# tsurumeso/vocal-remover

Hardware: NVIDIA H100
Metric: seconds-of-audio/sec separated (n_fft=2048, hop=1024) (higher is better)
Workload: dtype bf16x3 (split-bf16 operands hi+lo, 3 wgmma passes, fp32 accumulate); fft/lstm fp32

## Files before the change

### vocal-remover_b200/csrc/api.cu

```cuda
#include <stdio.h>
#include <string.h>

#include <string>

#include "../../include/vr_b200.h"
#include "engine.h"
#include "kernels.h"
#include "tc_plan.h"

struct vr_ctx {
  vr::Engine* eng;
  std::string err;
};

static std::string g_create_err;

static int fail(vr_ctx* c, const std::string& m) {
  if (c) c->err = m;
  return -1;
}
static int done(vr_ctx* c, bool ok) {
  if (ok) return 0;
  c->err = c->eng->err;
  return -1;
// ... 345 lines not shown
  return 0;
}

int64_t vr_launch_count(const vr_ctx* ctx) { return ctx && ctx->eng ? ctx->eng->launches : 0; }

int vr_profile_enable(vr_ctx* ctx, int32_t on) {
  CHECK_CTX(ctx);
  ctx->eng->profile_enable(on != 0);
  return 0;
}

int vr_profile_read(vr_ctx* ctx, double* out6) {
  CHECK_CTX(ctx);
  return done(ctx, ctx->eng->profile_read(out6));
}

int vr_profile_dump(vr_ctx* ctx, char* text, int64_t cap, int64_t* needed) {
  CHECK_CTX(ctx);
  std::string t;
  if (!ctx->eng->profile_dump(t)) return done(ctx, false);
  if (needed) *needed = (int64_t)t.size() + 1;
  if (text && cap > 0) {
    const size_t n = t.size() < (size_t)cap - 1 ? t.size() : (size_t)cap - 1;
    memcpy(text, t.data(), n);
    text[n] = 0;
  }
  return 0;
}

int vr_debug_conv(vr_ctx* ctx, const float* x, int32_t N, int32_t Cin, int32_t H, int32_t W, const float* w,
                  const float* bias, int32_t Cout, int32_t k, int32_t stride, int32_t dil_h, int32_t dil_w, int32_t act,
                  int32_t use_tc, float* y, void* stream) {
  CHECK_CTX(ctx);
  return done(ctx, ctx->eng->debug_conv(x, N, Cin, H, W, w, bias, Cout, k, stride, dil_h, dil_w, act, use_tc, y,
                                        (cudaStream_t)stream));
}

int vr_debug_decoder(vr_ctx* ctx, const float* low, int32_t N, int32_t Cl, int32_t h, int32_t w, const float* skip,
                     int32_t Cs, const float* wgt, const float* bias, int32_t Cout, int32_t act, int32_t fused, float* y,
                     void* stream) {
  CHECK_CTX(ctx);
  return done(ctx, ctx->eng->debug_decoder(low, N, Cl, h, w, skip, Cs, wgt, bias, Cout, act, fused, y,
                                           (cudaStream_t)stream));
}

int vr_debug_tensor(vr_ctx* ctx, const char* name, int32_t n0, int32_t n, float* out, int64_t* shape4, void* stream) {
  CHECK_NET(ctx);
  if (!name || !shape4) return fail(ctx, "vr_debug_tensor: name and shape4 are required");
  return done(ctx, ctx->eng->debug_tensor(name, n0, n, out, shape4, (cudaStream_t)stream));
}

int vr_debug_set(int32_t key, int32_t value) {
  int* knob = key == 0 ? &vr::g_debug.trace : key == 2 ? &vr::g_debug.rows_wide : key == 3 ? &vr::g_debug.halo
            : key == 6 ? &vr::g_debug.kskip : key == 7 ? &vr::g_debug.crop_mask : nullptr;
  if (!knob) return -1;
  *knob = value;
  return 0;
}

int64_t vr_debug_trace(uint64_t* host_out, int64_t capacity) {
  return vr::tc_rows_read_trace((unsigned long long*)host_out, (long long)capacity);
}

}
```

### vocal-remover_b200/csrc/conv_tc.cu

```cuda
#include <cuda.h>
#include <stdio.h>

#include <map>
#include <tuple>

#include "engine.h"
#include "tc_common.cuh"
#include "tc_plan.h"

namespace vr {

static constexpr int kMaxStages = 8;
static constexpr int kConsumerWarps = 8;
static constexpr int kThreads = 32 * kConsumerWarps + 32;
static constexpr int kStaticSmem = 2048;

struct TcParams {
  int N, Ho, Wo, Wt, Ht, Nt, tiles_w, tiles_h, m_tiles, n_tiles;
  int stride, pad_h, pad_w, dil_h, dil_w, KW;
  int cchunks, total_sub, CinPadTC, Cout, act, stages;
  bf16* out_hi;
  bf16* out_lo;
  int64_t osn, osh;
  int osw;
// ... 258 lines not shown

static unsigned long long weight_group_mask(const ConvLayer& L, const float* wp, int CinPad) {
  if (CinPad / 8 > 64) return ~0ull;
  unsigned long long m = 0x3ull;
  for (int ci = 0; ci < L.CinPad; ++ci) {
    bool any = false;
    for (int t = 0; t < L.k * L.k && !any; ++t)
      for (int co = 0; co < L.Cout && !any; ++co) any = wp[((size_t)t * L.CinPad + ci) * L.CoutPad + co] != 0.f;
    if (any) m |= 1ull << (ci / 8);
  }
  return m;
}

static bool encode_weight_map(TcConv& tc, int rows, int K, int box_rows, std::string& err, const std::string& name) {
  cuuint64_t dims[3] = {(cuuint64_t)K, (cuuint64_t)rows, 2};
  cuuint64_t strides[2] = {(cuuint64_t)K * 2, (cuuint64_t)rows * K * 2};
  cuuint32_t box[3] = {(cuuint32_t)tc.KB, (cuuint32_t)box_rows, 2};
  cuuint32_t es[3] = {1, 1, 1};
  CUresult r = tc_encode_fn()(&tc.map_b, CU_TENSOR_MAP_DATA_TYPE_BFLOAT16, 3, tc.w_planes.get(), dims, strides, box, es,
                              CU_TENSOR_MAP_INTERLEAVE_NONE, swizzle_for(tc.KB), CU_TENSOR_MAP_L2_PROMOTION_L2_256B,
                              CU_TENSOR_MAP_FLOAT_OOB_FILL_NONE);
  if (r != CUDA_SUCCESS) {
    err = "cuTensorMapEncodeTiled(weights) failed for " + name + " code " + std::to_string((int)r);
    return false;
  }
  return true;
}

const CUtensorMap* tc_activation_map(TcConv& tc, const ActView& v, int bw, int bh, int bn, int es, std::string& err,
                                     const std::string& name) {
  const ViewKey key = std::make_tuple((const void*)v.hi, (const void*)v.lo, v.N, v.H, v.W, v.C, bw, bh, bn);
  auto it = tc.map_a.find(key);
  if (it != tc.map_a.end()) return &it->second;
  const int64_t plane = (const char*)v.lo - (const char*)v.hi;
  if (v.sw % 8 || v.sh % 8 || v.sn % 8 || (reinterpret_cast<uintptr_t>(v.hi) & 15) || plane <= 0 || plane % 16) {
    err = "internal: the input of " + name + " is not 16-byte aligned or its lo plane does not follow its hi plane";
    return nullptr;
  }
  cuuint64_t dims[5] = {(cuuint64_t)v.C, (cuuint64_t)v.W, (cuuint64_t)v.H, (cuuint64_t)v.N, 2};
  cuuint64_t strides[4] = {(cuuint64_t)v.sw * 2, (cuuint64_t)v.sh * 2, (cuuint64_t)v.sn * 2, (cuuint64_t)plane};
  cuuint32_t box[5] = {(cuuint32_t)tc.KB, (cuuint32_t)bw, (cuuint32_t)bh, (cuuint32_t)bn, 2};
  cuuint32_t estr[5] = {1, (cuuint32_t)es, (cuuint32_t)es, 1, 1};
  CUtensorMap m;
  CUresult r = tc_encode_fn()(&m, CU_TENSOR_MAP_DATA_TYPE_BFLOAT16, 5, (void*)v.hi, dims, strides, box, estr,
                              CU_TENSOR_MAP_INTERLEAVE_NONE, swizzle_for(tc.KB), CU_TENSOR_MAP_L2_PROMOTION_L2_256B,
                              CU_TENSOR_MAP_FLOAT_OOB_FILL_NONE);
  if (r != CUDA_SUCCESS) {
    err = "cuTensorMapEncodeTiled(activations) failed for " + name + " code " + std::to_string((int)r);
    return nullptr;
  }
  return &tc.map_a.emplace(key, m).first->second;
}

bool tc_prepare(ConvLayer& L, const float* w, const float* b, int H, int W, bool rows_wide, std::string& err) {
  const TcKind kind = tc_choose(L, H, W, rows_wide);
  if (kind == TC_NONE) return true;
  if (!tc_encode_fn()) {
    err = "cuTensorMapEncodeTiled is not available from the driver";
    return false;
  }
  auto tc = std::make_shared<TcConv>();
  tc->kind = kind;
  tc->H = H; tc->W = W;
  const NTiling nt = n_tiling(L, kind == TC_ROWS, rows_wide);
  const int BN = nt.BN, cin16 = round_up(L.CinPad, 16);
  tc->BN = BN; tc->n_tiles = nt.n_tiles;
  tc->KB = kind != TC_GENERIC ? 32 : cin16 % 64 == 0 ? 64 : cin16 % 32 == 0 ? 32 : 16;
  const int CinPad = round_up(L.CinPad, tc->KB);
  tc->CinPad = CinPad;
  tc->chunks = CinPad / tc->KB;
  tc->kmask = weight_group_mask(L, w, CinPad);
  const int rows = nt.n_tiles * BN;
  std::vector<uint16_t> planes;
  int brows, K;
  if (kind == TC_ROWS) {
    brows = 3 * rows;
    K = 3 * CinPad;
    planes = split_bf16(L, w, brows, K, [&](int co, int t, int ci) {
      return (size_t)(co / BN * 3 * BN + (2 - t / 3) * BN + co % BN) * K + (size_t)(t % 3) * CinPad + ci;
    });
  } else {
    brows = rows;
    K = L.k * L.k * CinPad;
    planes = split_bf16(L, w, brows, K, [&](int co, int t, int ci) { return (size_t)co * K + (size_t)t * CinPad + ci; });
  }
  std::vector<float> bias((size_t)rows, 0.f);
  for (int co = 0; co < L.Cout; ++co) bias[(size_t)co] = b[co];
  if (tc->w_planes.alloc(planes.size() * 2) != cudaSuccess || tc->bias.alloc(bias.size() * 4) != cudaSuccess) {
    err = "cudaMalloc failed while packing tensor-core weights for " + L.name;
    return false;
  }
  if (!upload(tc->w_planes.get(), planes.data(), planes.size() * 2, err) ||
      !upload(tc->bias.get(), bias.data(), bias.size() * 4, err) ||
      !encode_weight_map(*tc, brows, K, kind == TC_ROWS ? 3 * BN : BN, err, L.name))
    return false;
  L.tc = tc;
  return true;
}

cudaError_t tc_launch(const ConvLayer& L, const ActView& in, const ActView& out, cudaStream_t s, std::string& err,
                      const ConvFusion& f) {
  TcConv& tc = *L.tc;
  if (out.H != tc.H || out.W != tc.W || (in.H - 1) / L.stride + 1 != out.H || (in.W - 1) / L.stride + 1 != out.W) {
    err = "internal: " + L.name + " is launched on maps of another size than it was prepared for";
    return cudaErrorInvalidValue;
  }
// ... 52 lines not shown
```

### vocal-remover_b200/csrc/conv_tc_rows.cu

```cuda
#include <stdio.h>

#include "engine.h"
#include "tc_common.cuh"
#include "tc_plan.h"

namespace vr {

static constexpr int kInterpWarps = 10;
static constexpr int kConsumerWarps = 8;
static constexpr int kTmaWarp = kConsumerWarps;
static constexpr int kInterpWarp0 = kConsumerWarps + 1;
__host__ __device__ constexpr int rows_per_tile(int BN) { return BN == 64 ? 2 : BN == 32 ? 4 : 8; }
static constexpr int kUpProducerWarps = 12;
static constexpr int kUpConsumerRegs = 128;
static constexpr int kUpProducerRegs = 72;
static constexpr int kUpLaunchRegs = 96;
static_assert(kConsumerWarps * kUpConsumerRegs + kUpProducerWarps * kUpProducerRegs <=
                  (kConsumerWarps + kUpProducerWarps) * kUpLaunchRegs,
              "setmaxnreg.inc would wait forever for registers the block does not own");
__host__ __device__ constexpr int rows_threads(bool up) { return 32 * (kConsumerWarps + (up ? kUpProducerWarps : 1)); }
static constexpr int kRowPx = 130;
static constexpr int kBoxPx = 136;
static constexpr int kMaxASlots = 8;
static constexpr int kStaticSmem = 3072;
static constexpr int kSrcPx = 68;
static constexpr uint32_t kKB = 32;
static constexpr uint32_t kRowB = kKB * 2;
static constexpr uint32_t kAPlane = kBoxPx * kRowB;
static constexpr uint32_t kASlot = 2 * kAPlane;

static constexpr int kTraceEvents = 2048;
__device__ unsigned long long g_rows_trace[3 * kTraceEvents * 3];

template <int BN>
struct RowsGeom {
  static constexpr uint32_t kBPlane = 3 * BN * kRowB;
  static constexpr uint32_t kBKw = 2 * kBPlane;
  static constexpr uint32_t kBBuf = 3 * kBKw;
};

struct RowsParams {
  int N, H, W, tiles_w, tiles_h, n_tiles, total_tiles;
  int col0;
  int chunks, CinPadR, Cout, act;
  int n_aslots;
  bf16* out_hi;
  bf16* out_lo;
  int64_t osn, osh;
  int osw;
  const float* bias;
  int up_chunks, xH, xW;
  const bf16* x_hi;
  const bf16* x_lo;
  int64_t xsn, xsh;
  int xsw;
  int trace;
  unsigned long long kmask;
  int a_c_off;
  int l_chunk;
  int n_uslots;
  float up_sh, up_sw;
  const float* dot_w;
  float* dot_out;
  MaskOutParams mask;
};

struct RowsTile {
  int nt, w0, h0, n;
};
template <int R>
__device__ __forceinline__ RowsTile rows_tile(const RowsParams& p, int tile) {
  RowsTile t;
  t.nt = tile % p.n_tiles;
  int mt = tile / p.n_tiles;
  t.w0 = p.col0 + (mt % p.tiles_w) * 128;
  mt /= p.tiles_w;
  t.h0 = (mt % p.tiles_h) * R;
  t.n = mt / p.tiles_h;
  return t;
}

struct RowsConsumer {
  MbarRing a_up, a_tma, b;
  HeldSlot held_b;
};

template <int BN, int R, int r>
__device__ __forceinline__ MbarRing consume_rows(MbarRing a, RowsConsumer& st, float* acc, uint32_t (&fr)[2][16],
                                                 uint32_t lrow, uint32_t bsrc, uint32_t dhi, uint32_t ksm, int lane) {
  constexpr int o_lo = r - 2 < 0 ? 0 : r - 2;
  constexpr int o_hi = r > R - 1 ? R - 1 : r;
  a.wait_full();
  const uint32_t row = lrow + (uint32_t)a.slot * kASlot;
#pragma unroll
  for (int kw = 0; kw < 3; ++kw) {
    uint32_t* f = fr[(3 * r + kw) & 1];
    const uint32_t q = (row >> 6) + (uint32_t)kw;
#pragma unroll
// ... 15 lines not shown
                            b_row + (RowsGeom<BN>::kBPlane >> 4), dhi);
      }
    }
    wg_commit();
    if (kw == 2) warp_arrive(a.empty(), lane);
    wg_wait<1>();
    st.held_b.release(st.b, lane);
  }
  a.advance();
  if constexpr (r + 1 < R + 2)
    return consume_rows<BN, R, r + 1>(a, st, acc, fr, lrow, bsrc, dhi, ksm, lane);
  else
    return a;
}

__device__ __forceinline__ float dot_pair(float v0, float v1, const float* bias_s, const float* dot_s, int c, float slope) {
  const float t0 = v0 + bias_s[c], t1 = v1 + bias_s[c + 1];
  return fmaf(fmaxf(t0, 0.f) + slope * fminf(t0, 0.f), dot_s[c], (fmaxf(t1, 0.f) + slope * fminf(t1, 0.f)) * dot_s[c + 1]);
}

template <int BN>
__device__ __forceinline__ void mask_pixel(const RowsParams& p, const float* v, const float* bias_s,
                                           const float* mask_s, float slope, int lane, int n, int bin, int w) {
  float x[BN / 4];
#pragma unroll
  for (int j = 0; j < BN / 8; ++j) {
    const int c = 8 * j + 2 * (lane & 3);
    const float t0 = v[4 * j] + bias_s[c], t1 = v[4 * j + 1] + bias_s[c + 1];
    const float y0 = fmaxf(t0, 0.f) + slope * fminf(t0, 0.f);
    const float y1 = fmaxf(t1, 0.f) + slope * fminf(t1, 0.f);
    const float2 hf = bf2_to_f2(f2_to_bf2(y0, y1));
    const float2 lf = bf2_to_f2(f2_to_bf2(y0 - hf.x, y1 - hf.y));
    x[2 * j] = hf.x + lf.x;
    x[2 * j + 1] = hf.y + lf.y;
  }
  const float* wm = mask_s + (lane & 1) * BN;
  float a = 0.f;
#pragma unroll
  for (int c = 0; c < BN; ++c)
    a = fmaf(__shfl_sync(0xffffffffu, x[2 * (c >> 3) + (c & 1)], (lane & ~3) | ((c >> 1) & 3)), wm[c], a);
  const float m = 1.f / (1.f + expf(-a));
  const int tr = w - p.col0;
  const int64_t t = p.mask.t_base0 + (int64_t)n * p.mask.roi_t + tr;
  const bool nyquist = (lane & 2) != 0;
  if (t < 0 || t >= p.mask.t_limit || (nyquist && bin != p.H - 1)) return;
  float* d = p.mask.out + (int64_t)n * p.mask.stride_n + (int64_t)(nyquist ? bin + 1 : bin) * p.mask.stride_bin +
             p.mask.t_base0 + tr + ((lane & 1) ? p.mask.stride_c : 0);
  *d = p.mask.accumulate ? (*d + m) * 0.5f : m;
}

template <int BN, bool UP>
__global__ void __launch_bounds__(rows_threads(UP), 1)
    conv_tc_rows_kernel(const __grid_constant__ CUtensorMap tmA, const __grid_constant__ CUtensorMap tmB,
                        const __grid_constant__ CUtensorMap tmL, const RowsParams p) {
  typedef RowsGeom<BN> G;
  constexpr int R = rows_per_tile(BN);
  extern __shared__ uint8_t smem_raw[];
  __shared__ __align__(8) uint64_t bar_afull[kMaxASlots];
  __shared__ __align__(8) uint64_t bar_aempty[kMaxASlots];
  __shared__ __align__(8) uint64_t bar_bfull[2];
  __shared__ __align__(8) uint64_t bar_bempty[2];
  __shared__ float bias_s[256];
  __shared__ float dot_s[256];

  const int warp = __shfl_sync(0xffffffffu, (int)threadIdx.x >> 5, 0);
  const int lane = threadIdx.x & 31;
  const uint32_t smem_base = (smem_u32(smem_raw) + 1023u) & ~1023u;
  const uint32_t a_base = smem_base;
  const uint32_t b_base = smem_base + (uint32_t)p.n_aslots * kASlot;
  MbarRing a_up(smem_u32(&bar_afull[0]), smem_u32(&bar_aempty[0]), 0, p.n_uslots);
  MbarRing a_tma(smem_u32(&bar_afull[0]), smem_u32(&bar_aempty[0]), p.n_uslots, p.n_aslots);
  MbarRing b_ring(smem_u32(&bar_bfull[0]), smem_u32(&bar_bempty[0]), 0, 2);

  if (warp == kTmaWarp && lane == 0) {
    tma_prefetch(&tmA);
    tma_prefetch(&tmB);
    a_up.init(kInterpWarps, kConsumerWarps);
    a_tma.init(1, kConsumerWarps);
    b_ring.init(1, kConsumerWarps);
    asm volatile("fence.mbarrier_init.release.cluster;" ::: "memory");
  }
  for (int i = threadIdx.x; i < p.n_tiles * BN; i += blockDim.x) {
    bias_s[i] = __ldg(p.bias + i);
    dot_s[i] = p.dot_out && i < p.Cout ? __ldg(p.dot_w + i) : 0.f;
  }
  constexpr bool kMaskable = UP && BN <= 32;
  if constexpr (kMaskable) {
    if (p.mask.out)
      for (int i = threadIdx.x; i < 2 * BN; i += blockDim.x) dot_s[i] = __ldg(p.mask.w + i);
  }
  __syncthreads();
  if (warp < kConsumerWarps) {
    if constexpr (UP) setmaxnreg_inc<kUpConsumerRegs>();
    const int wg = warp >> 2;
    const float slope = act_slope(p.act);
    const uint32_t dhi = desc_hi(8 * kRowB, 2u);
    const uint32_t lrow = a_base + (uint32_t)(64 * wg + 16 * (warp & 3) + (lane & 15)) * kRowB;
    RowsConsumer st{a_up, a_tma, b_ring};
    float acc[R * BN / 2];
    uint32_t fr[2][16];
    for (int tile = blockIdx.x; tile < p.total_tiles; tile += gridDim.x) {
#pragma unroll
      for (int i = 0; i < R * BN / 2; ++i) acc[i] = 0.f;
      for (int cc = 0; cc < p.chunks; ++cc) {
        st.b.wait_full();
        const uint32_t bsrc = desc_lo(b_base + (uint32_t)st.b.slot * G::kBBuf);
        const bool up = cc < p.up_chunks;
        const uint32_t gm = chunk_groups(p.kmask, cc);
        const uint32_t ksm = ((gm & 0x3u) ? 1u : 0u) | ((gm & 0xCu) ? 2u : 0u);
        const MbarRing a = consume_rows<BN, R, 0>(up ? st.a_up : st.a_tma, st, acc, fr, lrow, bsrc, dhi, ksm, lane);
        st.a_up.slot = up ? a.slot : st.a_up.slot;
        st.a_up.phase = up ? a.phase : st.a_up.phase;
        st.a_tma.slot = up ? st.a_tma.slot : a.slot;
        st.a_tma.phase = up ? st.a_tma.phase : a.phase;
        st.held_b.hold(st.b);
        st.b.advance();
      }
      wg_wait<0>();
      st.held_b.release_last(st.b, lane);

      const RowsTile tl = rows_tile<R>(p, tile);
      const int w0 = tl.w0, h0 = tl.h0, n = tl.n;
      const int c_lane = tl.nt * BN + 2 * (lane & 3);
#pragma unroll
      for (int orow = 0; orow < R; ++orow) {
#pragma unroll
        for (int hr = 0; hr < 2; ++hr) {
          const int px = 64 * wg + 16 * (warp & 3) + (lane >> 2) + 8 * hr;
          const float* v = acc + orow * (BN / 2) + 2 * hr;
          if constexpr (kMaskable) {
            if (p.mask.out) {
              mask_pixel<BN>(p, v, bias_s, dot_s, slope, lane, n, h0 + orow, w0 + px);
              continue;
            }
          }
          if (p.dot_out) {
            float d = 0.f;
#pragma unroll
            for (int j = 0; j < BN / 8; ++j) d += dot_pair(v[4 * j], v[4 * j + 1], bias_s, dot_s, c_lane + 8 * j, slope);
            d += __shfl_xor_sync(0xffffffffu, d, 1);
            d += __shfl_xor_sync(0xffffffffu, d, 2);
            if ((lane & 3) == 0) atomicAdd(p.dot_out + ((int64_t)n * p.H + (h0 + orow)) * p.W + (w0 + px), d);
          }
          const int64_t obase = (int64_t)n * p.osn + (int64_t)(h0 + orow) * p.osh + (int64_t)(w0 + px) * p.osw;
#pragma unroll
          for (int j = 0; j < BN / 8; ++j)
            epilogue_pair(v[4 * j], v[4 * j + 1], bias_s, c_lane + 8 * j, p.Cout, slope, p.out_hi + obase,
                          p.out_lo + obase);
        }
      }
    }
  } else {
    if constexpr (UP) setmaxnreg_dec<kUpProducerRegs>();
    if (warp == kTmaWarp) {
      if (elect_one_sync()) {
#ifdef VR_TRACE
        const bool tr = p.trace && blockIdx.x == 0;
#else
        constexpr bool tr = false;
#endif
        int tn = 0;
        for (int tile = blockIdx.x; tile < p.total_tiles; tile += gridDim.x) {
          const RowsTile tl = rows_tile<R>(p, tile);
          const int nt = tl.nt, w0 = tl.w0, h0 = tl.h0, n = tl.n;
          for (int cc = 0; cc < p.chunks; ++cc) {
            b_ring.wait_empty();
            const uint32_t bdst = b_base + (uint32_t)b_ring.slot * G::kBBuf;
            mbar_expect_tx(b_ring.full(), G::kBBuf);
#pragma unroll
            for (int kw = 0; kw < 3; ++kw)
              tma_load_3d(bdst + (uint32_t)kw * G::kBKw, &tmB, kw * p.CinPadR + cc * (int)kKB, nt * 3 * BN, 0,
                          b_ring.full());
            b_ring.advance();
            if (cc < p.up_chunks) continue;
            const bool from_l = cc == p.l_chunk;
            const int c0 = from_l ? 0 : cc * (int)kKB + p.a_c_off;
            for (int r = 0; r < R + 2; ++r) {
              const unsigned long long t0 = tr ? clock64() : 0ull;
              a_tma.wait_empty();
              mbar_expect_tx(a_tma.full(), kASlot);
              tma_load_5d(a_base + (uint32_t)a_tma.slot * kASlot, from_l ? &tmL : &tmA, c0, w0 - 1, h0 - 1 + r, n, 0,
                          a_tma.full());
              if (tr && tn < kTraceEvents) {
                g_rows_trace[(1 * kTraceEvents + tn) * 3 + 0] = t0;
                g_rows_trace[(1 * kTraceEvents + tn) * 3 + 1] = clock64();
                g_rows_trace[(1 * kTraceEvents + tn) * 3 + 2] = 0ull;
                ++tn;
              }
              a_tma.advance();
            }
          }
        }
      }
      __syncwarp();
    } else if (UP && warp < kInterpWarp0 + kInterpWarps) {
      if (p.up_chunks > 0) {
        const int wk = warp - kInterpWarp0;
        const int xi = lane >> 2, j = lane & 3;
        const int sx = 7 * wk + xi;
        const bool emit = xi < 7 && sx < kSrcPx;
        const float inv_sw = p.up_sw > 0.f ? 1.f / p.up_sw : 0.f;
#ifdef VR_TRACE
        const bool tr = p.trace && blockIdx.x == 0 && wk == 0;
#else
// ... 94 lines not shown
#pragma unroll
              for (int i = 0; i < 8; ++i) {
                const float t = __shfl_down_sync(0xffffffffu, v[i], 4);
                nv[i] = last_px ? v[i] : t;
              }
              const unsigned long long t1 = tr ? clock64() : 0ull;
              a_up.wait_empty();
              const unsigned long long t2 = tr ? clock64() : 0ull;
              uint8_t* slot = smem_raw + (a_base - smem_u32(smem_raw)) + (size_t)a_up.slot * kASlot;
#pragma unroll
              for (int k = 0; k < 3; ++k) {
                if (e_off[k] < 0) continue;
                const float lx = e_lx[k], hx = 1.f - lx;
                float y[8];
#pragma unroll
                for (int i = 0; i < 8; ++i) y[i] = hx * v[i] + lx * nv[i];
                bf16x8 oh, ol;
                split8(y, oh, ol);
                *reinterpret_cast<uint4*>(slot + e_off[k]) = oh;
                *reinterpret_cast<uint4*>(slot + kAPlane + e_off[k]) = ol;
              }
              if (z_off >= 0) {
                *reinterpret_cast<uint4*>(slot + z_off) = make_uint4(0, 0, 0, 0);
                *reinterpret_cast<uint4*>(slot + kAPlane + z_off) = make_uint4(0, 0, 0, 0);
              }
              warp_arrive(a_up.full(), lane);
              fetch();
              if (tr && lane == 0 && tn < kTraceEvents) {
                g_rows_trace[(2 * kTraceEvents + tn) * 3 + 0] = t0;
                g_rows_trace[(2 * kTraceEvents + tn) * 3 + 1] = t2 - t1;
                g_rows_trace[(2 * kTraceEvents + tn) * 3 + 2] = clock64();
              }
              ++tn;
              a_up.advance();
            }
          }
        }
      }
      }
  }
}

#define VR_ROWS_FOR_ALL(X) X(16, true) X(16, false) X(32, true) X(32, false) X(64, true) X(64, false)

static int rows_b_bytes(int BN) {
#define VR_ROWS_B(BN_, UP_) if (BN == BN_) return (int)(2 * RowsGeom<BN_>::kBBuf);
  VR_ROWS_FOR_ALL(VR_ROWS_B)
#undef VR_ROWS_B
  return 0;
}

bool tc_rows_has(int BN) { return rows_b_bytes(BN) > 0; }

cudaError_t tc_rows_launch(const ConvLayer& L, TcConv& tc, const ActView& in, const ActView& out, cudaStream_t s,
                           std::string& err, const ConvFusion& f) {
  const ActView* up_src = f.up;
  if (up_src && (!tc.fuses_upsample(up_src->C) || up_src->H * 2 != in.H || up_src->W * 2 != in.W || up_src->sw % 8)) {
    err = "tc_rows_launch: fused upsample needs a half-resolution source of 32k channels";
    return cudaErrorInvalidValue;
  }
  if (up_src && up_src->C + in.C > tc.CinPad) {
    err = "tc_rows_launch: with a fused upsample the input must hold only the channels after the up-sampled ones";
    return cudaErrorInvalidValue;
  }
  const ActView* last = f.last_chunk;
  if (last && (last->H != in.H || last->W != in.W || last->N != in.N || last->C > tc.KB)) {
    err = "tc_rows_launch: the last-chunk tensor must match the input geometry and fit one chunk";
    return cudaErrorInvalidValue;
  }
  const CUtensorMap* map_a = tc_activation_map(tc, in, kBoxPx, 1, 1, 1, err, L.name);
  const CUtensorMap* map_l = last ? tc_activation_map(tc, *last, kBoxPx, 1, 1, 1, err, L.name) : map_a;
  if (!map_a || !map_l) return cudaErrorInvalidValue;
  if (f.mask && !tc.fuses_mask(L.Cout, f.mask->offset, up_src != nullptr)) {
    err = "tc_rows_launch: the fused output layer needs a fused upsample, one N tile of Cout <= 32 channels and a "
          "kept width that is a multiple of 128";
    return cudaErrorInvalidValue;
  }
  const int col0 = f.mask ? f.mask->offset : 0;
  RowsParams p;
  p.N = out.N; p.H = out.H; p.W = out.W;
  const bool up = up_src != nullptr;
  p.col0 = col0;
  p.tiles_w = (out.W - 2 * col0) / 128; p.tiles_h = out.H / rows_per_tile(tc.BN); p.n_tiles = tc.n_tiles;
  p.total_tiles = p.tiles_w * p.tiles_h * out.N * tc.n_tiles;
  p.chunks = tc.chunks; p.CinPadR = tc.CinPad; p.Cout = L.Cout; p.act = L.act;
  p.out_hi = out.hi; p.out_lo = out.lo;
  p.osn = out.sn; p.osh = out.sh; p.osw = out.sw;
  p.bias = tc.bias.get();
  p.up_chunks = 0; p.xH = p.xW = 0;
  p.x_hi = p.x_lo = nullptr; p.xsn = p.xsh = 0; p.xsw = 0;
  p.trace = g_debug.trace == 1 ? 1 : 0;
  p.up_sh = p.up_sw = 0.f;
  p.dot_w = f.dot_w; p.dot_out = f.dot_w ? f.dot_out : nullptr;
  p.mask = f.mask ? *f.mask : MaskOutParams{};
  p.a_c_off = 0;
  p.l_chunk = last ? tc.chunks - 1 : -1;
  p.kmask = g_debug.kskip == 1 ? tc.kmask : ~0ull;
  if (up_src) {
    p.a_c_off = -up_src->C;
    p.up_chunks = up_src->C / 32;
    p.xH = up_src->H; p.xW = up_src->W;
    p.x_hi = up_src->hi; p.x_lo = up_src->lo;
    p.xsn = up_src->sn; p.xsh = up_src->sh; p.xsw = up_src->sw;
    if ((reinterpret_cast<uintptr_t>(up_src->hi) | reinterpret_cast<uintptr_t>(up_src->lo)) & 15) {
      err = "tc_rows_launch: upsample source planes must be 16-byte aligned";
      return cudaErrorInvalidValue;
    }
    p.up_sh = in.H > 1 ? (float)(up_src->H - 1) / (float)(in.H - 1) : 0.f;
    p.up_sw = in.W > 1 ? (float)(up_src->W - 1) / (float)(in.W - 1) : 0.f;
  }
  const TcDevice& dv = tc_device();
  if (!dv.ok) {
    err = "tc_rows_launch: cannot query the current device";
    return cudaErrorInvalidValue;
  }
  const int b_bytes = rows_b_bytes(tc.BN);
  p.n_aslots = (dv.max_smem - kStaticSmem - 1024 - b_bytes) / (int)kASlot;
  if (p.n_aslots > kMaxASlots) p.n_aslots = kMaxASlots;
  if (p.n_aslots < (p.up_chunks > 0 ? 4 : 2)) {
    err = "tc_rows_launch: shared memory too small";
    return cudaErrorInvalidValue;
  }
  p.n_uslots = p.up_chunks > 0 ? p.n_aslots - p.n_aslots / 2 : 0;
  if (p.up_chunks > 0 && p.n_aslots - p.n_uslots < 2) p.n_uslots = p.n_aslots - 2;
  const int dyn = p.n_aslots * (int)kASlot + b_bytes + 1024;
  const int grid = p.total_tiles < dv.num_sms ? p.total_tiles : dv.num_sms;
  const int threads = rows_threads(up);
#define VR_ROWS_LAUNCH(BN_, UP_)                                                              \
  if (tc.BN == BN_ && up == UP_) {                                                            \
    conv_tc_rows_kernel<BN_, UP_><<<grid, threads, dyn, s>>>(*map_a, tc.map_b, *map_l, p);    \
    return cudaGetLastError();                                                                \
  }
  VR_ROWS_FOR_ALL(VR_ROWS_LAUNCH)
#undef VR_ROWS_LAUNCH
  err = "tc_rows_launch: no kernel instantiation for this channel tile";
  return cudaErrorInvalidValue;
}


int tc_rows_read_trace(unsigned long long* out, long long capacity) {
  const long long n = 3LL * kTraceEvents * 3;
  if (capacity < n) return -1;
  if (cudaMemcpyFromSymbol(out, g_rows_trace, sizeof(unsigned long long) * (size_t)n) != cudaSuccess) return -1;
  return (int)n;
}

void tc_rows_set_attributes(int max_smem) {
#define VR_ROWS_SET(BN_, UP_)                                                                        \
  cudaFuncSetAttribute(conv_tc_rows_kernel<BN_, UP_>, cudaFuncAttributeMaxDynamicSharedMemorySize,   \
                       max_smem - kStaticSmem);                                                      \
  cudaFuncSetAttribute(conv_tc_rows_kernel<BN_, UP_>, cudaFuncAttributePreferredSharedMemoryCarveout, 100);
  VR_ROWS_FOR_ALL(VR_ROWS_SET)
#undef VR_ROWS_SET
}

}
```

### vocal-remover_b200/csrc/tc_common.cuh

```cuda
#pragma once
#include <cuda.h>
#include <stdint.h>
#include <stdio.h>

#include "common.cuh"

namespace vr {

__device__ __forceinline__ uint32_t smem_u32(const void* p) { return (uint32_t)__cvta_generic_to_shared(p); }

__device__ __forceinline__ bool elect_one_sync() {
  uint32_t pred;
  asm volatile(
      "{\n\t"
      ".reg .pred P1;\n\t"
      "elect.sync _|P1, 0xffffffff;\n\t"
      "selp.u32 %0, 1, 0, P1;\n\t"
      "}"
      : "=r"(pred));
  return pred != 0;
}

__device__ __forceinline__ void mbar_init(uint32_t bar, uint32_t count) {
  asm volatile("mbarrier.init.shared::cta.b64 [%0], %1;" ::"r"(bar), "r"(count));
}
__device__ __forceinline__ void mbar_expect_tx(uint32_t bar, uint32_t bytes) {
  asm volatile("mbarrier.arrive.expect_tx.shared::cta.b64 _, [%0], %1;" ::"r"(bar), "r"(bytes) : "memory");
}
__device__ __forceinline__ void mbar_arrive(uint32_t bar) {
  asm volatile("mbarrier.arrive.shared::cta.b64 _, [%0];" ::"r"(bar) : "memory");
}
__device__ __forceinline__ void mbar_wait(uint32_t bar, uint32_t parity) {
#ifdef VR_WAIT_TIMEOUT
  asm volatile(
      "{\n\t"
      ".reg .pred p, q;\n\t"
      ".reg .u32 n;\n\t"
      "mov.u32 n, 0;\n\t"
      "WAIT_LOOP:\n\t"
      "mbarrier.try_wait.parity.shared::cta.b64 p, [%0], %1;\n\t"
      "@p bra WAIT_DONE;\n\t"
      "add.u32 n, n, 1;\n\t"
      "setp.lt.u32 q, n, 0x10000000;\n\t"
      "@q bra WAIT_LOOP;\n\t"
      "trap;\n\t"
      "WAIT_DONE:\n\t"
      "}" ::"r"(bar),
      "r"(parity)
      : "memory");
#else
  asm volatile(
      "{\n\t"
      ".reg .pred p;\n\t"
      "WAIT_LOOP:\n\t"
      "mbarrier.try_wait.parity.shared::cta.b64 p, [%0], %1;\n\t"
      "@p bra WAIT_DONE;\n\t"
      "bra WAIT_LOOP;\n\t"
      "WAIT_DONE:\n\t"
      "}" ::"r"(bar),
      "r"(parity)
      : "memory");
#endif
// ... 225 lines not shown
  static __device__ __forceinline__ void mma(float* d, const uint32_t* a, uint64_t b) {
    asm volatile(
        "wgmma.mma_async.sync.aligned.m64n128k16.f32.bf16.bf16 {%0, %1, %2, %3, %4, %5, %6, %7, %8, %9, %10, %11, %12, %13, %14, %15, %16, %17, %18, %19, %20, %21, %22, %23, %24, %25, %26, %27, %28, %29, %30, %31, %32, %33, %34, %35, %36, %37, %38, %39, %40, %41, %42, %43, %44, %45, %46, %47, %48, %49, %50, %51, %52, %53, %54, %55, %56, %57, %58, %59, %60, %61, %62, %63}, {%64, %65, %66, %67}, %68, 1, 1, 1, 0;"
        : "+f"(d[0]), "+f"(d[1]), "+f"(d[2]), "+f"(d[3]), "+f"(d[4]), "+f"(d[5]), "+f"(d[6]), "+f"(d[7]), "+f"(d[8]), "+f"(d[9]), "+f"(d[10]), "+f"(d[11]), "+f"(d[12]), "+f"(d[13]), "+f"(d[14]), "+f"(d[15]), "+f"(d[16]), "+f"(d[17]), "+f"(d[18]), "+f"(d[19]), "+f"(d[20]), "+f"(d[21]), "+f"(d[22]), "+f"(d[23]), "+f"(d[24]), "+f"(d[25]), "+f"(d[26]), "+f"(d[27]), "+f"(d[28]), "+f"(d[29]), "+f"(d[30]), "+f"(d[31]), "+f"(d[32]), "+f"(d[33]), "+f"(d[34]), "+f"(d[35]), "+f"(d[36]), "+f"(d[37]), "+f"(d[38]), "+f"(d[39]), "+f"(d[40]), "+f"(d[41]), "+f"(d[42]), "+f"(d[43]), "+f"(d[44]), "+f"(d[45]), "+f"(d[46]), "+f"(d[47]), "+f"(d[48]), "+f"(d[49]), "+f"(d[50]), "+f"(d[51]), "+f"(d[52]), "+f"(d[53]), "+f"(d[54]), "+f"(d[55]), "+f"(d[56]), "+f"(d[57]), "+f"(d[58]), "+f"(d[59]), "+f"(d[60]), "+f"(d[61]), "+f"(d[62]), "+f"(d[63])
        : "r"(a[0]), "r"(a[1]), "r"(a[2]), "r"(a[3]), "l"(b)
        : "memory");
  }
};
template <int N>
__device__ __forceinline__ void wgmma_split3_rs(float* d, const uint32_t* a_hi, const uint32_t* a_lo, uint32_t b_hi,
                                                uint32_t b_lo, uint32_t dhi) {
  WgmmaRS<N>::mma(d, a_hi, desc64(b_hi, dhi));
  WgmmaRS<N>::mma(d, a_lo, desc64(b_hi, dhi));
  WgmmaRS<N>::mma(d, a_hi, desc64(b_lo, dhi));
}

__device__ __forceinline__ void ldsm_x4(uint32_t* r, uint32_t addr) {
  asm volatile("ldmatrix.sync.aligned.m8n8.x4.shared.b16 {%0, %1, %2, %3}, [%4];"
               : "=r"(r[0]), "=r"(r[1]), "=r"(r[2]), "=r"(r[3])
               : "r"(addr)
               : "memory");
}

template <int N>
__device__ __forceinline__ void setmaxnreg_inc() {
  asm volatile("setmaxnreg.inc.sync.aligned.u32 %0;" ::"n"(N));
}
template <int N>
__device__ __forceinline__ void setmaxnreg_dec() {
  asm volatile("setmaxnreg.dec.sync.aligned.u32 %0;" ::"n"(N));
}

__device__ __forceinline__ float act_slope(int act) { return act == ACT_RELU ? 0.f : act == ACT_LEAKY ? 0.01f : 1.f; }

__device__ __forceinline__ void epilogue_pair(float v0, float v1, const float* bias_s, int c, int Cout, float slope,
                                              bf16* out_hi, bf16* out_lo) {
  if (c >= Cout) return;
  const float t0 = v0 + bias_s[c], t1 = v1 + bias_s[c + 1];
  const float y0 = fmaxf(t0, 0.f) + slope * fminf(t0, 0.f);
  const float y1 = fmaxf(t1, 0.f) + slope * fminf(t1, 0.f);
  bf16* h = out_hi + c;
  bf16* l = out_lo + c;
  if (c + 1 < Cout && ((reinterpret_cast<uintptr_t>(h) | reinterpret_cast<uintptr_t>(l)) & 3) == 0) {
    const uint32_t uh = f2_to_bf2(y0, y1);
    const float2 hf = bf2_to_f2(uh);
    *reinterpret_cast<uint32_t*>(h) = uh;
    *reinterpret_cast<uint32_t*>(l) = f2_to_bf2(y0 - hf.x, y1 - hf.y);
  } else {
    split_bf16(y0, h[0], l[0]);
    if (c + 1 < Cout) split_bf16(y1, h[1], l[1]);
  }
}

__device__ __forceinline__ uint32_t chunk_groups(unsigned long long kmask, int cc) {
  const int sh = cc * 4;
  return sh + 4 <= 64 ? (uint32_t)(kmask >> sh) & 0xFu : 0xFu;
}

__device__ __forceinline__ void tma_load_4d(uint32_t dst, const CUtensorMap* map, int c0, int c1, int c2, int c3,
                                            uint32_t bar) {
  asm volatile(
      "cp.async.bulk.tensor.4d.shared::cluster.global.tile.mbarrier::complete_tx::bytes [%0], [%1, {%2, %3, %4, %5}], "
      "[%6];" ::"r"(dst),
      "l"(map), "r"(c0), "r"(c1), "r"(c2), "r"(c3), "r"(bar)
      : "memory");
}

}
```

### vocal-remover_b200/csrc/tc_plan.h

```cpp
#pragma once
#include <cuda.h>

#include <map>
#include <tuple>

#include "engine.h"

namespace vr {

enum TcKind {
  TC_NONE,
  TC_GENERIC,
  TC_ROWS,
  TC_HALO,
};

typedef std::tuple<const void*, const void*, int, int, int, int, int, int, int> ViewKey;

struct TcConv {
  TcKind kind = TC_NONE;
  int H = 0, W = 0;
  int KB = 0, CinPad = 0, chunks = 0, BN = 0, n_tiles = 0;
  unsigned long long kmask = ~0ull;
  DevPtr<bf16> w_planes;
  DevPtr<float> bias;
  CUtensorMap map_b;
  std::map<ViewKey, CUtensorMap> map_a;
  bool fuses_upsample(int up_C) const { return kind == TC_ROWS && up_C % 32 == 0 && up_C <= CinPad; }
  bool fuses_dot() const { return kind == TC_ROWS; }
  bool fuses_mask(int Cout, int offset, bool up) const {
    const int kept = W - 2 * offset;
    return kind == TC_ROWS && up && n_tiles == 1 && BN <= 32 && BN == Cout && offset >= 0 && kept > 0 &&
           kept % 128 == 0;
  }
};

TcKind tc_choose(const ConvLayer& L, int H, int W, bool rows_wide);
const CUtensorMap* tc_activation_map(TcConv& tc, const ActView& v, int bw, int bh, int bn, int es, std::string& err,
                                     const std::string& name);

cudaError_t tc_rows_launch(const ConvLayer& L, TcConv& tc, const ActView& in, const ActView& out, cudaStream_t s,
                           std::string& err, const ConvFusion& f);
void tc_rows_set_attributes(int max_smem);
bool tc_rows_has(int BN);
int tc_rows_read_trace(unsigned long long* out, long long capacity);

cudaError_t tc_halo_launch(const ConvLayer& L, TcConv& tc, const ActView& in, const ActView& out, cudaStream_t s,
                           std::string& err);
void tc_halo_set_attributes(int max_smem);
bool tc_halo_has(int BN);

struct TcDevice {
  bool ok = false;
  int num_sms = 0, max_smem = 0;
};
const TcDevice& tc_device();

struct TcDebug {
  int trace = 0;
  int rows_wide = 0;
  int halo = 0;
  int kskip = 1;
  int crop_mask = 1;
};
extern TcDebug g_debug;

}
```

Measured before the change: 2888.

## Stage rows-conv epilogue through swizzled shared memory and store via TMA

For small-N rows conv tiles (BN 16/32), consumer warps now write the bias+activation+bf16 hi/lo split into per-warp swizzled shared-memory buffers and issue TMA tensor stores, replacing scattered global stores. It double-buffers with bulk async groups and reserves shared memory for staging, which reduces the A-slot ring depth. The goal is coalesced, asynchronous output writes that overlap the next tile's MMA, at the cost of fewer pipeline slots and extra fences.

```diff
diff --git a/vocal-remover_b200/csrc/api.cu b/vocal-remover_b200/csrc/api.cu
--- a/vocal-remover_b200/csrc/api.cu
+++ b/vocal-remover_b200/csrc/api.cu
@@ -421,7 +421,8 @@
 
 int vr_debug_set(int32_t key, int32_t value) {
   int* knob = key == 0 ? &vr::g_debug.trace : key == 2 ? &vr::g_debug.rows_wide : key == 3 ? &vr::g_debug.halo
-            : key == 6 ? &vr::g_debug.kskip : key == 7 ? &vr::g_debug.crop_mask : nullptr;
+            : key == 6 ? &vr::g_debug.kskip : key == 7 ? &vr::g_debug.crop_mask
+            : key == 8 ? &vr::g_debug.rows_staged : nullptr;
   if (!knob) return -1;
   *knob = value;
   return 0;
diff --git a/vocal-remover_b200/csrc/conv_tc.cu b/vocal-remover_b200/csrc/conv_tc.cu
--- a/vocal-remover_b200/csrc/conv_tc.cu
+++ b/vocal-remover_b200/csrc/conv_tc.cu
@@ -334,6 +334,37 @@
   return &tc.map_a.emplace(key, m).first->second;
 }
 
+bool tc_output_addressable(const ActView& v) {
+  const int64_t plane = (const char*)v.lo - (const char*)v.hi;
+  return v.sw % 8 == 0 && v.sh % 8 == 0 && v.sn % 8 == 0 && (reinterpret_cast<uintptr_t>(v.hi) & 15) == 0 && plane > 0 &&
+         plane % 16 == 0;
+}
+
+const CUtensorMap* tc_output_map(TcConv& tc, const ActView& v, int C, int bc, int bw, int bh, std::string& err,
+                                 const std::string& name) {
+  const ViewKey key = std::make_tuple((const void*)v.hi, (const void*)v.lo, v.N, v.H, v.W, C, bc, bw, bh);
+  auto it = tc.map_out.find(key);
+  if (it != tc.map_out.end()) return &it->second;
+  if (!tc_output_addressable(v)) {
+    err = "internal: the output of " + name + " is not 16-byte aligned or its lo plane does not follow its hi plane";
+    return nullptr;
+  }
+  cuuint64_t dims[5] = {(cuuint64_t)C, (cuuint64_t)v.W, (cuuint64_t)v.H, (cuuint64_t)v.N, 2};
+  cuuint64_t strides[4] = {(cuuint64_t)v.sw * 2, (cuuint64_t)v.sh * 2, (cuuint64_t)v.sn * 2,
+                           (cuuint64_t)((const char*)v.lo - (const char*)v.hi)};
+  cuuint32_t box[5] = {(cuuint32_t)bc, (cuuint32_t)bw, (cuuint32_t)bh, 1, 2};
+  cuuint32_t estr[5] = {1, 1, 1, 1, 1};
+  CUtensorMap m;
+  CUresult r = tc_encode_fn()(&m, CU_TENSOR_MAP_DATA_TYPE_BFLOAT16, 5, (void*)v.hi, dims, strides, box, estr,
+                              CU_TENSOR_MAP_INTERLEAVE_NONE, swizzle_for(bc), CU_TENSOR_MAP_L2_PROMOTION_L2_256B,
+                              CU_TENSOR_MAP_FLOAT_OOB_FILL_NONE);
+  if (r != CUDA_SUCCESS) {
+    err = "cuTensorMapEncodeTiled(output) failed for " + name + " code " + std::to_string((int)r);
+    return nullptr;
+  }
+  return &tc.map_out.emplace(key, m).first->second;
+}
+
 bool tc_prepare(ConvLayer& L, const float* w, const float* b, int H, int W, bool rows_wide, std::string& err) {
   const TcKind kind = tc_choose(L, H, W, rows_wide);
   if (kind == TC_NONE) return true;
diff --git a/vocal-remover_b200/csrc/conv_tc_rows.cu b/vocal-remover_b200/csrc/conv_tc_rows.cu
--- a/vocal-remover_b200/csrc/conv_tc_rows.cu
+++ b/vocal-remover_b200/csrc/conv_tc_rows.cu
@@ -32,11 +32,25 @@
 static constexpr int kTraceEvents = 2048;
 __device__ unsigned long long g_rows_trace[3 * kTraceEvents * 3];
 
-template <int BN>
+__host__ __device__ constexpr int rows_store_rows(int BN, bool up) {
+  return BN == 16 ? rows_per_tile(16) : BN == 32 ? (up ? 1 : rows_per_tile(32)) : 0;
+}
+__host__ __device__ constexpr bool rows_staged(int BN, bool up) { return rows_store_rows(BN, up) > 0; }
+__host__ __device__ constexpr int rows_stage_bufs(int BN, bool up) {
+  return rows_store_rows(BN, up) == rows_per_tile(BN) ? 1 : 2;
+}
+
+template <int BN, bool UP = false>
 struct RowsGeom {
   static constexpr uint32_t kBPlane = 3 * BN * kRowB;
   static constexpr uint32_t kBKw = 2 * kBPlane;
   static constexpr uint32_t kBBuf = 3 * kBKw;
+  static constexpr uint32_t kOutPxB = BN * 2;
+  static constexpr int kStoreRows = rows_store_rows(BN, UP);
+  static constexpr int kStageBufs = rows_stage_bufs(BN, UP);
+  static constexpr uint32_t kStagePlane = (uint32_t)(kStoreRows > 0 ? kStoreRows : 1) * 16 * kOutPxB;
+  static constexpr uint32_t kStageBuf = 2 * kStagePlane;
+  static constexpr uint32_t kStageBytes = rows_staged(BN, UP) ? kConsumerWarps * kStageBufs * kStageBuf : 0;
 };
 
 struct RowsParams {
@@ -44,6 +58,7 @@
   int col0;
   int chunks, CinPadR, Cout, act;
   int n_aslots;
+  int staged;
   bf16* out_hi;
   bf16* out_lo;
   int64_t osn, osh;
@@ -165,8 +180,9 @@
 template <int BN, bool UP>
 __global__ void __launch_bounds__(rows_threads(UP), 1)
     conv_tc_rows_kernel(const __grid_constant__ CUtensorMap tmA, const __grid_constant__ CUtensorMap tmB,
-                        const __grid_constant__ CUtensorMap tmL, const RowsParams p) {
-  typedef RowsGeom<BN> G;
+                        const __grid_constant__ CUtensorMap tmL, const __grid_constant__ CUtensorMap tmO,
+                        const RowsParams p) {
+  typedef RowsGeom<BN, UP> G;
   constexpr int R = rows_per_tile(BN);
   extern __shared__ uint8_t smem_raw[];
   __shared__ __align__(8) uint64_t bar_afull[kMaxASlots];
@@ -181,6 +197,7 @@
   const uint32_t smem_base = (smem_u32(smem_raw) + 1023u) & ~1023u;
   const uint32_t a_base = smem_base;
   const uint32_t b_base = smem_base + (uint32_t)p.n_aslots * kASlot;
+  const uint32_t stage_base = b_base + 2 * G::kBBuf;
   MbarRing a_up(smem_u32(&bar_afull[0]), smem_u32(&bar_aempty[0]), 0, p.n_uslots);
   MbarRing a_tma(smem_u32(&bar_afull[0]), smem_u32(&bar_aempty[0]), p.n_uslots, p.n_aslots);
   MbarRing b_ring(smem_u32(&bar_bfull[0]), smem_u32(&bar_bempty[0]), 0, 2);
@@ -188,6 +205,7 @@
   if (warp == kTmaWarp && lane == 0) {
     tma_prefetch(&tmA);
     tma_prefetch(&tmB);
+    if (rows_staged(BN, UP) && p.staged) tma_prefetch(&tmO);
     a_up.init(kInterpWarps, kConsumerWarps);
     a_tma.init(1, kConsumerWarps);
     b_ring.init(1, kConsumerWarps);
@@ -212,7 +230,16 @@
     RowsConsumer st{a_up, a_tma, b_ring};
     float acc[R * BN / 2];
     uint32_t fr[2][16];
+    const bool staged = rows_staged(BN, UP) && p.staged;
+#ifdef VR_TRACE
+    const bool tr = p.trace && blockIdx.x == 0 && threadIdx.x == 0;
+    int tn = 0;
+    unsigned long long t_tile = 0ull, t_epi = 0ull;
+#endif
     for (int tile = blockIdx.x; tile < p.total_tiles; tile += gridDim.x) {
+#ifdef VR_TRACE
+      if (tr) t_tile = clock64();
+#endif
 #pragma unroll
       for (int i = 0; i < R * BN / 2; ++i) acc[i] = 0.f;
       for (int cc = 0; cc < p.chunks; ++cc) {
@@ -231,12 +258,22 @@
       }
       wg_wait<0>();
       st.held_b.release_last(st.b, lane);
+#ifdef VR_TRACE
+      if (tr) t_epi = clock64();
+#endif
 
       const RowsTile tl = rows_tile<R>(p, tile);
       const int w0 = tl.w0, h0 = tl.h0, n = tl.n;
       const int c_lane = tl.nt * BN + 2 * (lane & 3);
 #pragma unroll
       for (int orow = 0; orow < R; ++orow) {
+        constexpr int SR = G::kStoreRows > 0 ? G::kStoreRows : 1;
+        const int sr = orow % SR;
+        const uint32_t sbuf = stage_base + (uint32_t)(warp * G::kStageBufs + (orow / SR) % G::kStageBufs) * G::kStageBuf;
+        if (staged && sr == 0) {
+          if (lane_id() == 0) bulk_wait_read<G::kStageBufs - 1>();
+          __syncwarp();
+        }
 #pragma unroll
         for (int hr = 0; hr < 2; ++hr) {
           const int px = 64 * wg + 16 * (warp & 3) + (lane >> 2) + 8 * hr;
@@ -255,14 +292,40 @@
             d += __shfl_xor_sync(0xffffffffu, d, 2);
             if ((lane & 3) == 0) atomicAdd(p.dot_out + ((int64_t)n * p.H + (h0 + orow)) * p.W + (w0 + px), d);
           }
+          if (staged) {
+            const uint32_t spx = (uint32_t)(16 * sr + (lane_id() >> 2) + 8 * hr);
+            const uint32_t sc = (uint32_t)(lane_id() & 3) * 4u;
+#pragma unroll
+            for (int j = 0; j < BN / 8; ++j)
+              stage_pair(v[4 * j], v[4 * j + 1], bias_s, c_lane + 8 * j, slope,
+                         sbuf + swizzled_offset<G::kOutPxB>(spx, 16u * j + sc), G::kStagePlane);
+            continue;
+          }
           const int64_t obase = (int64_t)n * p.osn + (int64_t)(h0 + orow) * p.osh + (int64_t)(w0 + px) * p.osw;
 #pragma unroll
           for (int j = 0; j < BN / 8; ++j)
             epilogue_pair(v[4 * j], v[4 * j + 1], bias_s, c_lane + 8 * j, p.Cout, slope, p.out_hi + obase,
                           p.out_lo + obase);
         }
+        if (staged && sr == SR - 1) {
+          fence_proxy_async_shared();
+          __syncwarp();
+          if (lane_id() == 0) {
+            tma_store_5d(&tmO, sbuf, tl.nt * BN, w0 + 64 * wg + 16 * (warp & 3), h0 + orow - (SR - 1), n, 0);
+            bulk_commit();
+          }
+        }
       }
+#ifdef VR_TRACE
+      if (tr && tn < kTraceEvents) {
+        g_rows_trace[tn * 3 + 0] = t_tile;
+        g_rows_trace[tn * 3 + 1] = t_epi;
+        g_rows_trace[tn * 3 + 2] = clock64();
+        ++tn;
+      }
+#endif
     }
+    if (staged && lane_id() == 0) bulk_wait<0>();
   } else {
     if constexpr (UP) setmaxnreg_dec<kUpProducerRegs>();
     if (warp == kTmaWarp) {
@@ -463,6 +526,13 @@
 
 bool tc_rows_has(int BN) { return rows_b_bytes(BN) > 0; }
 
+static int rows_stage_bytes(int BN, bool up) {
+#define VR_ROWS_S(BN_, UP_) if (BN == BN_ && up == UP_) return (int)RowsGeom<BN_, UP_>::kStageBytes;
+  VR_ROWS_FOR_ALL(VR_ROWS_S)
+#undef VR_ROWS_S
+  return 0;
+}
+
 cudaError_t tc_rows_launch(const ConvLayer& L, TcConv& tc, const ActView& in, const ActView& out, cudaStream_t s,
                            std::string& err, const ConvFusion& f) {
   const ActView* up_src = f.up;
@@ -526,7 +596,11 @@
     return cudaErrorInvalidValue;
   }
   const int b_bytes = rows_b_bytes(tc.BN);
-  p.n_aslots = (dv.max_smem - kStaticSmem - 1024 - b_bytes) / (int)kASlot;
+  p.staged = rows_stage_bytes(tc.BN, up) > 0 && g_debug.rows_staged == 1 && !f.mask && tc_output_addressable(out) ? 1 : 0;
+  const int stage_bytes = p.staged ? rows_stage_bytes(tc.BN, up) : 0;
+  const CUtensorMap* map_o = p.staged ? tc_output_map(tc, out, L.Cout, tc.BN, 16, rows_store_rows(tc.BN, up), err, L.name) : map_a;
+  if (!map_o) return cudaErrorInvalidValue;
+  p.n_aslots = (dv.max_smem - kStaticSmem - 1024 - b_bytes - stage_bytes) / (int)kASlot;
   if (p.n_aslots > kMaxASlots) p.n_aslots = kMaxASlots;
   if (p.n_aslots < (p.up_chunks > 0 ? 4 : 2)) {
     err = "tc_rows_launch: shared memory too small";
@@ -534,12 +608,12 @@
   }
   p.n_uslots = p.up_chunks > 0 ? p.n_aslots - p.n_aslots / 2 : 0;
   if (p.up_chunks > 0 && p.n_aslots - p.n_uslots < 2) p.n_uslots = p.n_aslots - 2;
-  const int dyn = p.n_aslots * (int)kASlot + b_bytes + 1024;
+  const int dyn = p.n_aslots * (int)kASlot + b_bytes + stage_bytes + 1024;
   const int grid = p.total_tiles < dv.num_sms ? p.total_tiles : dv.num_sms;
   const int threads = rows_threads(up);
 #define VR_ROWS_LAUNCH(BN_, UP_)                                                              \
   if (tc.BN == BN_ && up == UP_) {                                                            \
-    conv_tc_rows_kernel<BN_, UP_><<<grid, threads, dyn, s>>>(*map_a, tc.map_b, *map_l, p);    \
+    conv_tc_rows_kernel<BN_, UP_><<<grid, threads, dyn, s>>>(*map_a, tc.map_b, *map_l, *map_o, p); \
     return cudaGetLastError();                                                                \
   }
   VR_ROWS_FOR_ALL(VR_ROWS_LAUNCH)
diff --git a/vocal-remover_b200/csrc/tc_common.cuh b/vocal-remover_b200/csrc/tc_common.cuh
--- a/vocal-remover_b200/csrc/tc_common.cuh
+++ b/vocal-remover_b200/csrc/tc_common.cuh
@@ -8,6 +8,12 @@
 namespace vr {
 
 __device__ __forceinline__ uint32_t smem_u32(const void* p) { return (uint32_t)__cvta_generic_to_shared(p); }
+
+__device__ __forceinline__ int lane_id() {
+  int l;
+  asm volatile("mov.u32 %0, %%laneid;" : "=r"(l));
+  return l;
+}
 
 __device__ __forceinline__ bool elect_one_sync() {
   uint32_t pred;
@@ -339,6 +345,44 @@
   }
 }
 
+__device__ __forceinline__ void stage_pair(float v0, float v1, const float* bias_s, int c, float slope, uint32_t dst,
+                                           uint32_t lo_off) {
+  const float t0 = v0 + bias_s[c], t1 = v1 + bias_s[c + 1];
+  const float y0 = fmaxf(t0, 0.f) + slope * fminf(t0, 0.f);
+  const float y1 = fmaxf(t1, 0.f) + slope * fminf(t1, 0.f);
+  const uint32_t uh = f2_to_bf2(y0, y1);
+  const float2 hf = bf2_to_f2(uh);
+  const uint32_t ul = f2_to_bf2(y0 - hf.x, y1 - hf.y);
+  asm volatile("st.shared.b32 [%0], %1;" ::"r"(dst), "r"(uh) : "memory");
+  asm volatile("st.shared.b32 [%0], %1;" ::"r"(dst + lo_off), "r"(ul) : "memory");
+}
+
+template <int ROW_BYTES>
+__device__ __forceinline__ uint32_t swizzled_offset(uint32_t row, uint32_t b) {
+  const uint32_t off = row * ROW_BYTES + b;
+  return off ^ (((off >> 7) & (uint32_t)(ROW_BYTES / 16 - 1)) << 4);
+}
+
+__device__ __forceinline__ void tma_store_5d(const CUtensorMap* map, uint32_t src, int c0, int c1, int c2, int c3,
+                                             int c4) {
+  asm volatile(
+      "cp.async.bulk.tensor.5d.global.shared::cta.bulk_group [%0, {%2, %3, %4, %5, %6}], [%1];" ::"l"(map), "r"(src),
+      "r"(c0), "r"(c1), "r"(c2), "r"(c3), "r"(c4)
+      : "memory");
+}
+__device__ __forceinline__ void bulk_commit() { asm volatile("cp.async.bulk.commit_group;" ::: "memory"); }
+template <int N>
+__device__ __forceinline__ void bulk_wait_read() {
+  asm volatile("cp.async.bulk.wait_group.read %0;" ::"n"(N) : "memory");
+}
+template <int N>
+__device__ __forceinline__ void bulk_wait() {
+  asm volatile("cp.async.bulk.wait_group %0;" ::"n"(N) : "memory");
+}
+__device__ __forceinline__ void fence_proxy_async_shared() {
+  asm volatile("fence.proxy.async.shared::cta;" ::: "memory");
+}
+
 __device__ __forceinline__ uint32_t chunk_groups(unsigned long long kmask, int cc) {
   const int sh = cc * 4;
   return sh + 4 <= 64 ? (uint32_t)(kmask >> sh) & 0xFu : 0xFu;
diff --git a/vocal-remover_b200/csrc/tc_plan.h b/vocal-remover_b200/csrc/tc_plan.h
--- a/vocal-remover_b200/csrc/tc_plan.h
+++ b/vocal-remover_b200/csrc/tc_plan.h
@@ -26,6 +26,7 @@
   DevPtr<float> bias;
   CUtensorMap map_b;
   std::map<ViewKey, CUtensorMap> map_a;
+  std::map<ViewKey, CUtensorMap> map_out;
   bool fuses_upsample(int up_C) const { return kind == TC_ROWS && up_C % 32 == 0 && up_C <= CinPad; }
   bool fuses_dot() const { return kind == TC_ROWS; }
   bool fuses_mask(int Cout, int offset, bool up) const {
@@ -38,6 +39,9 @@
 TcKind tc_choose(const ConvLayer& L, int H, int W, bool rows_wide);
 const CUtensorMap* tc_activation_map(TcConv& tc, const ActView& v, int bw, int bh, int bn, int es, std::string& err,
                                      const std::string& name);
+bool tc_output_addressable(const ActView& v);
+const CUtensorMap* tc_output_map(TcConv& tc, const ActView& v, int C, int bc, int bw, int bh, std::string& err,
+                                 const std::string& name);
 
 cudaError_t tc_rows_launch(const ConvLayer& L, TcConv& tc, const ActView& in, const ActView& out, cudaStream_t s,
                            std::string& err, const ConvFusion& f);
@@ -62,6 +66,7 @@
   int halo = 0;
   int kskip = 1;
   int crop_mask = 1;
+  int rows_staged = 1;
 };
 extern TcDebug g_debug;
 
```

After: 2974 (median of 6 runs). 3.0% higher.
